# david-westreicher/minispark

Measured on AMD Instinct MI355X. Metric: TPC-H Q1 lineitem rows/sec, higher is better.
Workload: dtype f64

## Files before the change

minispark_amd/csrc/hs_agg_kernel.h:

```cpp
#pragma once

#include "hs_device.h"


typedef float hs_f32x4 __attribute__((ext_vector_type(4)));
typedef int hs_i32x4 __attribute__((ext_vector_type(4)));
typedef unsigned long long hs_u64x2 __attribute__((ext_vector_type(2)));

struct AggUnitArgs {
    hs_col key;
    hs_agg_spec spec;
    int32_t group_cap;
    int32_t hashed;
    int32_t batch;
    int32_t pad;
    const int64_t* unit_chunk0;
    const uint64_t* part_keys;
    const int64_t* part_rep;
    const uint64_t* part_acc;
    int64_t* out_rep;
    uint64_t* out_acc;
    int32_t* out_ngroups;
    uint32_t* flags;
    uint8_t* slab;
// ... 274 lines not shown
            const float4 v = *reinterpret_cast<const float4*>((const float*)c.data + row0);
            cell[0] = hs_d2u((double)v.x);
            cell[1] = hs_d2u((double)v.y);
            cell[2] = hs_d2u((double)v.z);
            cell[3] = hs_d2u((double)v.w);
            break;
        }
        case HS_I64:
        case HS_F64: {
            const ulonglong2 v0 = *reinterpret_cast<const ulonglong2*>((const uint64_t*)c.data + row0);
            const ulonglong2 v1 = *reinterpret_cast<const ulonglong2*>((const uint64_t*)c.data + row0 + 2);
            cell[0] = v0.x;
            cell[1] = v0.y;
            cell[2] = v1.x;
            cell[3] = v1.y;
            break;
        }
        case HS_U8: {
            const uint32_t v = *reinterpret_cast<const uint32_t*>((const uint8_t*)c.data + row0);
            cell[0] = v & 0xff;
            cell[1] = (v >> 8) & 0xff;
            cell[2] = (v >> 16) & 0xff;
            cell[3] = v >> 24;
            break;
        }
        case HS_I64_FOR16: {
            const uint2 v = *reinterpret_cast<const uint2*>((const uint16_t*)c.data + row0);
            const uint64_t b = (uint64_t)c.offs[0], s = (uint64_t)c.offs[1];
            cell[0] = b + (uint64_t)(v.x & 0xffff) * s;
            cell[1] = b + (uint64_t)(v.x >> 16) * s;
            cell[2] = b + (uint64_t)(v.y & 0xffff) * s;
            cell[3] = b + (uint64_t)(v.y >> 16) * s;
            break;
        }
        case HS_F32_LUT8: {
            const uint32_t v = *reinterpret_cast<const uint32_t*>((const uint8_t*)c.data + row0);
            const float* lut = (const float*)c.offs;
            const uint32_t last = (uint32_t)c.fixed_len - 1;
            cell[0] = hs_d2u((double)lut[min(v & 0xff, last)]);
            cell[1] = hs_d2u((double)lut[min((v >> 8) & 0xff, last)]);
            cell[2] = hs_d2u((double)lut[min((v >> 16) & 0xff, last)]);
            cell[3] = hs_d2u((double)lut[min(v >> 24, last)]);
            break;
        }
        case HS_STR:
            if (c.fixed_len == 1) hs_load_packed_quad<1>(c, row0, cell);
            else if (c.fixed_len == 2) hs_load_packed_quad<2>(c, row0, cell);
            else if (c.fixed_len == 4) hs_load_packed_quad<4>(c, row0, cell);
            break;
        default: break;
    }
}

struct AggCtx {
    int64_t row0;
    bool alive[HS_V];
    int slot[HS_V];
    uint64_t* dkeys;
    int64_t* dreps;
    uint64_t* tbl;
    uint8_t* dmap;
    uint32_t tid, nthr, mask;
    int32_t n_acc;
    uint32_t err;
    HsSpecBits sb;

    __device__ __forceinline__ int find_byte(const hs_col& key_col, uint64_t k, int64_t row, bool& live) {
        if (mask >= 255u) return find<false>(key_col, k, row, live);
        int s = 0;
        if (live) {
            const uint32_t b = (uint32_t)k & 0xffu;
            s = dmap[b];
            if (s == 0xff) {
                s = hs_dict_upsert_word(dkeys, dreps, mask, k, row);
                if (s < 0) {
                    err |= HS_FLAG_DICT_FULL;
                    live = false;
                    s = 0;
                } else {
                    dmap[b] = (uint8_t)s;
                }
            }
        }
        return s;
    }

    template <bool HASHED>
    __device__ __forceinline__ int find(const hs_col& key_col, uint64_t k, int64_t row, bool& live) {
        int s = 0;
        if (live) {
            if constexpr (HASHED) s = hs_dict_upsert_rows(dreps, mask, key_col, k, row);
            else s = hs_dict_upsert_word(dkeys, dreps, mask, k, row);
            if (s < 0) {
                err |= HS_FLAG_DICT_FULL;
                live = false;
                s = 0;
            }
        }
        return s;
    }

    __device__ __forceinline__ void fold(const hs_agg_spec& spec, uint32_t a, int s, bool live, uint64_t x) {
        if (live) {
            const uint32_t idx = ((uint32_t)s * (uint32_t)n_acc + a) * nthr + tid;
            (void)spec;
            tbl[idx] = hs_acc_fold(hs_spec_op(sb, a), hs_spec_int(sb, a), tbl[idx], x);
        }
    }

    template <int NA, int A, int OP, bool IS_INT>
    __device__ __forceinline__ void fold_c(int s, bool live, uint64_t x) {
        const uint32_t idx = ((uint32_t)(live ? s : 0) * (uint32_t)NA + (uint32_t)A) * nthr + tid;
        const uint64_t v = live ? x : hs_acc_identity(OP, IS_INT);
        tbl[idx] = hs_acc_fold(OP, IS_INT, tbl[idx], v);
    }
};

template <bool HASHED_, int D>
struct InterpProg {
    static constexpr bool HASHED = HASHED_;
    static constexpr bool TWO_STAGE = false;
    static constexpr bool STATIC_SPEC = false;
    static constexpr int NA = 0;
    static constexpr bool HAS_TABLES = false;
    struct Tables {};
    static __device__ constexpr uint32_t acc_op(int) { return 0; }
    static __device__ constexpr bool acc_int(int) { return false; }
    struct Cells {
        uint64_t cell[HS_FUSED_COLS][HS_V];
    };

    static __device__ __forceinline__ void load(const AggMainArgs& A, int64_t base, Cells& x) {
        const int ncols = A.cols.n < HS_FUSED_COLS ? A.cols.n : HS_FUSED_COLS;
#pragma unroll
        for (int c = 0; c < HS_FUSED_COLS; ++c) {
            if (c < ncols) {
                const hs_col& col = A.cols.c[c];
                if (col.kind != HS_STR || (c == A.key_col && hs_str_preloads(col))) hs_load_quad(col, base, x.cell[c]);
            }
        }
    }

    template <class Ctx>
    struct Sink {
        const AggMainArgs& A;
        const Cells& x;
        Ctx& ctx;
        __device__ __forceinline__ Sink(const AggMainArgs& a, const Cells& c, Ctx& k) : A(a), x(c), ctx(k) {}
        __device__ __forceinline__ void load(uint32_t s, uint64_t (&dst)[HS_V]) const {
            switch (s) {
#define HS_CASE(K)                                                          \
    case K:                                                                 \
        _Pragma("unroll") for (int j = 0; j < HS_V; ++j) dst[j] = x.cell[K][j]; \
        break;
                HS_CASE(0) HS_CASE(1) HS_CASE(2) HS_CASE(3) HS_CASE(4) HS_CASE(5) HS_CASE(6) HS_CASE(7)
#undef HS_CASE
                default: break;
            }
        }
        __device__ __forceinline__ uint64_t load(uint32_t s, int j) const {
            uint64_t tmp[HS_V];
            load(s, tmp);
            return tmp[j];
        }
        __device__ __forceinline__ bool live(int j) const { return ctx.alive[j]; }
        __device__ __forceinline__ int64_t row(int j) const { return ctx.row0 + j; }
        __device__ __forceinline__ void filter(int j, bool keep) { ctx.alive[j] = ctx.alive[j] && keep; }
        __device__ __forceinline__ void out(uint32_t, int, uint64_t) {}
        __device__ __forceinline__ void key() {
            const hs_col& kc = A.cols.c[A.key_col];
            uint64_t kcell[HS_V];
            const bool pre = (kc.kind != HS_STR) || hs_str_preloads(kc);
            if (pre) load((uint32_t)A.key_col, kcell);
            uint64_t ucell[HS_V] = {0, 0, 0, 0};
            if (A.unit_col >= 0) load((uint32_t)A.unit_col, ucell);
#pragma unroll
            for (int j = 0; j < HS_V; ++j) {
// ... 91 lines not shown
    extern __shared__ __align__(16) uint64_t hs_lds[];
    const uint32_t tid = threadIdx.x, nthr = blockDim.x;
    const int GC = A.group_cap;
    const int NA = A.spec.n_acc;
    uint64_t* dkeys = hs_lds;
    int64_t* dreps = (int64_t*)(hs_lds + GC);
    uint64_t* tbl = hs_lds + 2 * GC;

    const int64_t chunk = blockIdx.x;
    HS_SCAN_STAMP(0);
    if (A.stamps && threadIdx.x == 0)
        A.stamps[chunk * 16 + 7] = ((int64_t)__builtin_amdgcn_s_getreg((32 - 1) << 11 | 20) << 32) |
                                  (int64_t)(uint32_t)__builtin_amdgcn_s_getreg((32 - 1) << 11 | 4);
    const hs_chunk desc = A.chunks[chunk];
    const int64_t us = desc.unit_begin, c0 = desc.row_begin, c1 = desc.row_end;
    const int64_t stride = (int64_t)nthr * HS_V;
    int64_t base = c0 + (int64_t)tid * HS_V;
    typename Prog::Cells cur, nxt;
    if (base < c1) Prog::load(A, base, nxt);
    typename Prog::Tables tv;
    if constexpr (Prog::HAS_TABLES) Prog::load_tables(A, tid, tv);
    const HsSpecBits sb = hs_spec_bits(A.spec);

    __shared__ uint32_t s_overflowed;
    if (threadIdx.x == 0) s_overflowed = __hip_atomic_load(A.flags, __ATOMIC_RELAXED, __HIP_MEMORY_SCOPE_AGENT) & HS_FLAG_DICT_FULL;
    for (int i = tid; i < GC; i += nthr) {
        dkeys[i] = HS_EMPTY_KEY;
        dreps[i] = -1;
    }
    __shared__ uint8_t s_dmap[256];
    for (int i = tid; i < 256; i += nthr) s_dmap[i] = 0xff;
    for (int cellid = 0; cellid < GC * NA; ++cellid)
        tbl[(uint32_t)cellid * nthr + tid] = hs_acc_identity(hs_spec_op(sb, cellid % NA), hs_spec_int(sb, cellid % NA));
    if constexpr (Prog::HAS_TABLES) Prog::store_tables(tv, tid);
    __syncthreads();
    HS_SCAN_STAMP(1);
    if (s_overflowed) {
        for (int i = threadIdx.x; i < A.group_cap; i += blockDim.x) {
            hs_st_part(&A.part_keys[chunk * A.group_cap + i], HS_EMPTY_KEY);
            hs_st_part(&A.part_rep[chunk * A.group_cap + i], (int64_t)-1);
        }
    } else {
    AggCtx ctx;
    ctx.dkeys = dkeys;
    ctx.dreps = dreps;
    ctx.tbl = tbl;
    ctx.dmap = s_dmap;
    ctx.tid = tid;
    ctx.nthr = nthr;
    ctx.mask = (uint32_t)GC - 1;
    ctx.n_acc = NA;
    ctx.err = 0;
    ctx.sb = sb;
    HS_SCAN_STAMP(2);

    while (base < c1) {
        cur = nxt;
        const int64_t next_base = base + stride;
        if (next_base < c1) Prog::load(A, next_base, nxt);
        ctx.row0 = base;
#pragma unroll
        for (int j = 0; j < HS_V; ++j) {
            const int64_t r = base + j;
            ctx.alive[j] = (r >= us) && (r < c1);
            ctx.slot[j] = 0;
        }
        Prog::run(A, cur, ctx);
        base = next_base;
    }
    HS_SCAN_STAMP(3);
    __syncthreads();
    HS_SCAN_STAMP(14);

    const uint32_t wave = (uint32_t)__builtin_amdgcn_readfirstlane((int)(tid / HS_WAVE)), lane = tid % HS_WAVE, nwaves = nthr / HS_WAVE;
    if constexpr (Prog::STATIC_SPEC && (Prog::NA > 0)) {
        constexpr int SNA = Prog::NA;
        for (uint32_t sl = wave; sl < (uint32_t)GC; sl += nwaves) {
            if (__builtin_amdgcn_readfirstlane((int)(dreps[sl] >= 0)) == 0) continue;
            uint64_t v[SNA], t[SNA];
#pragma unroll
            for (int a = 0; a < SNA; ++a) v[a] = hs_acc_identity(Prog::acc_op(a), Prog::acc_int(a));
            for (uint32_t t0 = lane; t0 < nthr; t0 += HS_WAVE) {
#pragma unroll
                for (int a = 0; a < SNA; ++a) t[a] = tbl[(sl * (uint32_t)SNA + (uint32_t)a) * nthr + t0];
#pragma unroll
                for (int a = 0; a < SNA; ++a) v[a] = hs_acc_fold(Prog::acc_op(a), Prog::acc_int(a), v[a], t[a]);
            }
#pragma unroll
            for (int d = HS_WAVE / 2; d >= 1; d >>= 1) {
#pragma unroll
                for (int a = 0; a < SNA; ++a) t[a] = hs_shfl_down64(v[a], d);
#pragma unroll
                for (int a = 0; a < SNA; ++a) v[a] = hs_acc_fold(Prog::acc_op(a), Prog::acc_int(a), v[a], t[a]);
            }
            if (lane == 0) {
#pragma unroll
                for (int a = 0; a < SNA; ++a) hs_st_part(&A.part_acc[((int64_t)chunk * GC + sl) * SNA + a], v[a]);
            }
        }
    } else {
    constexpr int HS_RED = 6;
    const uint32_t ncells = (uint32_t)(GC * NA);
    for (uint32_t c0id = wave; c0id < ncells; c0id += nwaves * HS_RED) {
        uint64_t v[HS_RED], t[HS_RED];
        uint32_t ops[HS_RED];
        bool ints[HS_RED], on[HS_RED];
#pragma unroll
        for (int k = 0; k < HS_RED; ++k) {
            const uint32_t cellid = c0id + (uint32_t)k * nwaves;
            on[k] = cellid < ncells && __builtin_amdgcn_readfirstlane((int)(dreps[cellid < ncells ? cellid / NA : 0] >= 0)) != 0;
            const uint32_t a = on[k] ? cellid % NA : 0;
            ops[k] = hs_spec_op(sb, a);
            ints[k] = hs_spec_int(sb, a);
            v[k] = hs_acc_identity(ops[k], ints[k]);
        }
        for (uint32_t t0 = lane; t0 < nthr; t0 += HS_WAVE) {
#pragma unroll
            for (int k = 0; k < HS_RED; ++k) t[k] = on[k] ? tbl[(c0id + (uint32_t)k * nwaves) * nthr + t0] : 0ull;
#pragma unroll
            for (int k = 0; k < HS_RED; ++k)
                if (on[k]) v[k] = hs_acc_fold(ops[k], ints[k], v[k], t[k]);
// ... 446 lines not shown
```

minispark_amd/csrc/hs_jit.hip:

```cpp
#include <hip/hip_runtime.h>
#include <hip/hiprtc.h>
#include <stdarg.h>
#include <stdio.h>
#include <stdlib.h>
#include <string.h>

#include <chrono>
#include <mutex>
#include <string>
#include <sys/stat.h>
#include <unistd.h>

#include <unordered_map>
#include <vector>

#include "hs_agg_kernel.h"
#include "hs_embed.inc"

void hs_set_error(const char* fmt, ...);

namespace {

struct JitEntry {
    hipModule_t module = nullptr;
    hipFunction_t fn = nullptr;
    bool failed = false;
};

std::mutex g_mu;
std::unordered_map<std::string, JitEntry> g_cache;
int g_enabled = -1;
int g_compiled = 0, g_launches = 0, g_failures = 0;
std::string g_last_log;

bool jit_enabled() {
    if (g_enabled < 0) {
        const char* e = getenv("HIPSPARK_JIT");
        g_enabled = (e && e[0] == '0') ? 0 : 1;
    }
    return g_enabled != 0;
}

void appendf(std::string& s, const char* fmt, ...) {
    char buf[512];
    va_list ap;
    va_start(ap, fmt);
    vsnprintf(buf, sizeof(buf), fmt, ap);
    va_end(ap);
    s += buf;
}

bool slot_preloaded(const AggMainArgs& A, int c) {
    if (c >= A.cols.n || c >= HS_FUSED_COLS) return false;
    const hs_col& col = A.cols.c[c];
    if (col.kind != HS_STR) return true;
    return c == A.key_col && (col.fixed_len == 1 || col.fixed_len == 2 || col.fixed_len == 4);
}

int lut_entries(const hs_col& col) {
    int n = 16;
    while (n < col.fixed_len && n < 256) n *= 2;
    return n;
}

std::string cache_key(const AggMainArgs& A, bool hashed, bool shared, int nthr, bool scalar = false) {
    std::string k;
    int dev = 0;
    (void)hipGetDevice(&dev);
    appendf(k, "d%d|", dev);
    appendf(k, "v13|s%d|h%d|n%d|k%d|u%d|w%d|", shared ? 1 : scalar ? 2 : 0, hashed ? 1 : 0, A.cols.n, A.key_col, A.unit_col, shared ? 0 : nthr);
    for (int c = 0; c < A.cols.n; ++c) {
        const hs_col& col = A.cols.c[c];
        int fl = -1;
        if (col.kind == HS_STR && (col.fixed_len == 1 || col.fixed_len == 2 || col.fixed_len == 4) && c == A.key_col)
            fl = col.fixed_len;
        if (col.kind == HS_F32_LUT8) fl = lut_entries(col);
        appendf(k, "c%d:%d:%d|", c, col.kind, fl);
    }
    appendf(k, "a%d|", A.spec.n_acc);
    for (int a = 0; a < A.spec.n_acc; ++a) appendf(k, "%d%d", A.spec.op[a], A.spec.is_int[a]);
    k += "|";
    for (uint32_t i = 0; i < A.prog.n_ins; ++i) appendf(k, "%llx,", (unsigned long long)A.prog.ins[i]);
    return k;
}

std::string packed_cell_expr(const hs_col& col, int slot) {
    std::string e;

    if (col.kind == HS_U8) appendf(e, "((x.c%d_w[0] >> (8 * j)) & 0xffu)", slot);
    else if (col.fixed_len == 1) appendf(e, "((1ull << 56) | ((x.c%d_w[0] >> (8 * j)) & 0xffu))", slot);
    else if (col.fixed_len == 2) appendf(e, "((2ull << 56) | ((x.c%d_w[j >> 1] >> (16 * (j & 1))) & 0xffffu))", slot);
    else appendf(e, "((4ull << 56) | x.c%d_w[j])", slot);
    return e;
}

std::string ld_expr(const AggMainArgs& A, int slot) {
    std::string e;
    switch (A.cols.c[slot].kind & ~HS_PAIR) {
        case HS_I32: appendf(e, "(unsigned long long)(long long)x.c%d[j]", slot); break;
        case HS_F32: appendf(e, "hs_d2u((double)x.c%d[j])", slot); break;
        case HS_U8: e = "(unsigned long long)" + packed_cell_expr(A.cols.c[slot], slot); break;
        case HS_I64_FOR16:
            appendf(e, "(for%d_b + (unsigned long long)((unsigned)(x.c%d_q >> (16 * j)) & 0xffffu) * for%d_s)", slot, slot, slot);
            break;
        case HS_F32_LUT8:
            appendf(e, "hs_d2u(hs_lut_c%d[(x.c%d_w[0] >> (8 * j)) & %uu])", slot, slot, (unsigned)lut_entries(A.cols.c[slot]) - 1);
            break;
        case HS_JOIN8_CODE: e = "(unsigned long long)vb[j]"; break;
        case HS_JOIN8_UNIT: e = "(unsigned long long)vu[j]"; break;
        default: appendf(e, "x.c%d[j]", slot); break;
    }
    return e;
}


bool generate(const AggMainArgs& A, bool hashed, std::string& src, std::string& why, bool shared = false, int nthr = 256,
              bool scalar = false) {
    if (scalar && (shared || hashed || A.key_col >= 0 || A.unit_col >= 0)) {
        why = "the keyless kernel takes no key, unit column or shared table";
        return false;
    }
    const int NA = A.spec.n_acc;
    std::vector<std::string> agg_value((size_t)(NA > 0 ? NA : 0));
    const char* LD4 = "__builtin_nontemporal_load";
    std::string cells, loads, key_loads, join_prologue, body, hoisted, pair_keys, pair_take;
    std::string tables, table_regs, table_load, table_init;
    int j8_code = -1, j8_unit = -1, j8_src = -1;
    for (int c = 0; c < A.cols.n && c < HS_FUSED_COLS; ++c) {
        if (!slot_preloaded(A, c)) continue;
        const hs_col& col = A.cols.c[c];
        switch (col.kind) {
            case HS_I32:
                appendf(cells, "    int c%d[4];\n", c);
                appendf(loads, "    { const hs_i32x4 v = %s(reinterpret_cast<const hs_i32x4*>((const int*)A.cols.c[%d].data + base)); "
                               "x.c%d[0] = v.x; x.c%d[1] = v.y; x.c%d[2] = v.z; x.c%d[3] = v.w; }\n", LD4, c, c, c, c, c);
                break;
            case HS_F32:
                appendf(cells, "    float c%d[4];\n", c);
                appendf(loads, "    { const hs_f32x4 v = %s(reinterpret_cast<const hs_f32x4*>((const float*)A.cols.c[%d].data + base)); "
                               "x.c%d[0] = v.x; x.c%d[1] = v.y; x.c%d[2] = v.z; x.c%d[3] = v.w; }\n", LD4, c, c, c, c, c);
                break;
            case HS_I64:
            case HS_F64:
                appendf(cells, "    unsigned long long c%d[4];\n", c);
                appendf(loads, "    { const hs_u64x2 v0 = %s(reinterpret_cast<const hs_u64x2*>((const unsigned long long*)A.cols.c[%d].data + base)); "
                               "const hs_u64x2 v1 = %s(reinterpret_cast<const hs_u64x2*>((const unsigned long long*)A.cols.c[%d].data + base + 2)); "
                               "x.c%d[0] = v0.x; x.c%d[1] = v0.y; x.c%d[2] = v1.x; x.c%d[3] = v1.y; }\n", LD4, c, LD4, c, c, c, c, c);
                break;
            case HS_U8:
                appendf(cells, "    unsigned c%d_w[1];\n", c);
                appendf(loads, "    x.c%d_w[0] = *reinterpret_cast<const unsigned*>((const unsigned char*)A.cols.c[%d].data + base);\n", c, c);
                break;
            case HS_I64_FOR16:
            case HS_F32_LUT8:
                if (shared || c == A.key_col || c == A.unit_col || !col.offs || (col.kind == HS_F32_LUT8 && (col.fixed_len < 1 || col.fixed_len > 256))) {
                    why = "narrow columns are argument slots of the private-table and keyless tiers";
                    return false;
                }
                if (col.kind == HS_I64_FOR16) {
                    appendf(cells, "    unsigned long long c%d_q;\n", c);
                    appendf(loads, "    x.c%d_q = %s(reinterpret_cast<const unsigned long long*>((const unsigned short*)A.cols.c[%d].data + base));\n", c, LD4, c);
                    appendf(tables, "__shared__ unsigned long long hs_for_c%d[2];\n", c);
                    appendf(table_regs, "    unsigned long long for%d;\n", c);
                    appendf(table_load, "    t.for%d = (unsigned long long)A.cols.c[%d].offs[tid & 1u];\n", c, c);
                    appendf(table_init, "    if (tid < 2) hs_for_c%d[tid] = t.for%d;\n", c, c);
                    appendf(hoisted, "    const unsigned long long for%d_b = hs_for_c%d[0], for%d_s = hs_for_c%d[1];\n", c, c, c, c);
                } else {
                    const int entries = lut_entries(col);
                    appendf(cells, "    unsigned c%d_w[1];\n", c);
                    appendf(loads, "    x.c%d_w[0] = %s(reinterpret_cast<const unsigned*>((const unsigned char*)A.cols.c[%d].data + base));\n", c, LD4, c);
                    appendf(tables, "__shared__ double hs_lut_c%d[%d];\n", c, entries);
                    for (int k = 0; k * nthr < entries; ++k) {
                        appendf(table_regs, "    float lut%d_%d;\n", c, k);
                        appendf(table_load, "    t.lut%d_%d = ((const float*)A.cols.c[%d].offs)[min(tid + %du, (unsigned)A.cols.c[%d].fixed_len - 1u)];\n",
                                c, k, c, (unsigned)(k * nthr), c);
                        appendf(table_init, "    if (tid + %du < %du) hs_lut_c%d[tid + %du] = (double)t.lut%d_%d;\n", (unsigned)(k * nthr),
                                (unsigned)entries, c, (unsigned)(k * nthr), c, k);
                    }
                }
                break;
            case HS_STR:
                appendf(cells, "    unsigned c%d_w[%d];\n", c, col.fixed_len);
                if (col.fixed_len == 1)
                    appendf(loads, "    x.c%d_w[0] = *reinterpret_cast<const unsigned*>((const unsigned char*)A.cols.c[%d].data + base);\n", c, c);
                else if (col.fixed_len == 2)
                    appendf(loads, "    { const uint2 v = *reinterpret_cast<const uint2*>((const unsigned char*)A.cols.c[%d].data + base * 2); "
                                   "x.c%d_w[0] = v.x; x.c%d_w[1] = v.y; }\n", c, c, c);
                else
                    appendf(loads, "    { const uint4 v = *reinterpret_cast<const uint4*>((const unsigned char*)A.cols.c[%d].data + base * 4); "
                                   "x.c%d_w[0] = v.x; x.c%d_w[1] = v.y; x.c%d_w[2] = v.z; x.c%d_w[3] = v.w; }\n", c, c, c, c, c);
                break;
            case HS_JOIN8_CODE:
            case HS_JOIN8_UNIT:
                if (col.kind == HS_JOIN8_CODE) j8_code = c; else j8_unit = c;
                j8_src = c;
                break;
            case HS_PAIR | HS_I32:
            case HS_PAIR | HS_F32:
            case HS_PAIR | HS_I64: {
                if (!shared || c == A.key_col) {
                    why = "HS_PAIR columns are argument slots of the shared tier";
                    return false;
                }
                const int base = col.kind & ~HS_PAIR;
                const char* ty = base == HS_I32 ? "int" : base == HS_F32 ? "float" : "unsigned long long";
                appendf(cells, "    %s c%d[4];\n    long long ix%d[4];\n", ty, c, c);
                appendf(pair_keys, "    { const hs_u64x2 i0 = %s(reinterpret_cast<const hs_u64x2*>(A.cols.c[%d].offs + base)); "
                                   "const hs_u64x2 i1 = %s(reinterpret_cast<const hs_u64x2*>(A.cols.c[%d].offs + base + 2));\n"
                                   "      x.ix%d[0] = (long long)i0.x; x.ix%d[1] = (long long)i0.y; x.ix%d[2] = (long long)i1.x; "
                                   "x.ix%d[3] = (long long)i1.y; }\n", LD4, c, LD4, c, c, c, c, c);
                appendf(loads, "    { const %s* d = (const %s*)A.cols.c[%d].data; x.c%d[0] = d[x.ix%d[0]]; x.c%d[1] = d[x.ix%d[1]]; "
                               "x.c%d[2] = d[x.ix%d[2]]; x.c%d[3] = d[x.ix%d[3]]; }\n", ty, ty, c, c, c, c, c, c, c, c, c);
                appendf(pair_take, "    x.ix%d[0] = k.ix%d[0]; x.ix%d[1] = k.ix%d[1]; x.ix%d[2] = k.ix%d[2]; x.ix%d[3] = k.ix%d[3];\n",
                        c, c, c, c, c, c, c, c);
                break;
            }
            default:
                why = "unsupported column kind";
                return false;
        }
    }
    if (j8_src >= 0) {
        if (!shared || A.unit_col != j8_unit || j8_unit < 0 || !A.join.table) {
            why = "HS_JOIN8_* columns need the shared tier with the HS_JOIN8_UNIT column as unit column";
            return false;
        }
        cells += "    int jk[4];\n    unsigned jb[4];\n";
        appendf(key_loads, "    { const hs_i32x4 kv = %s(reinterpret_cast<const hs_i32x4*>((const int*)A.cols.c[%d].data + base));\n"
                           "      x.jk[0] = kv.x; x.jk[1] = kv.y; x.jk[2] = kv.z; x.jk[3] = kv.w; }\n", LD4, j8_src);
        loads += "    x.jb[0] = hs_join8_lookup(A.join, x.jk[0]);\n";
        loads += "    x.jb[1] = x.jk[1] != x.jk[0] ? hs_join8_lookup(A.join, x.jk[1]) : 0u;\n";
        loads += "    x.jb[2] = x.jk[2] != x.jk[1] ? hs_join8_lookup(A.join, x.jk[2]) : 0u;\n";
        loads += "    x.jb[3] = x.jk[3] != x.jk[2] ? hs_join8_lookup(A.join, x.jk[3]) : 0u;\n";
        join_prologue += "    unsigned vb[4], vu[4];\n    { const int np = A.join.n_parts;\n      const double inv = 1.0 / (double)np;\n";
        join_prologue += "      vb[0] = x.jb[0];\n      vu[0] = vb[0] == 0xffu ? 0xffu : hs_py_partition_inv(x.jk[0], np, inv);\n";
        for (int j = 1; j < 4; ++j) {
            appendf(join_prologue, "      { const bool same = x.jk[%d] == x.jk[%d];\n        vb[%d] = same ? vb[%d] : x.jb[%d];\n", j, j - 1, j, j - 1, j);
            appendf(join_prologue, "        vu[%d] = same ? vu[%d] : (vb[%d] == 0xffu ? 0xffu : hs_py_partition_inv(x.jk[%d], np, inv)); }\n", j, j - 1, j, j);
        }
        join_prologue += "    }\n";
    }
    key_loads += pair_keys;
    if (cells.empty()) cells = "    int unused;\n";

    std::vector<std::string> st;
    int tmp = 0;
    bool have_key = false;
    auto push_tmp = [&](const std::string& expr) {
        appendf(body, "        const unsigned long long t%d = %s;\n", tmp, expr.c_str());
        std::string name;
        appendf(name, "t%d", tmp++);
        st.push_back(name);
    };
    for (uint32_t pc = 0; pc < A.prog.n_ins; ++pc) {
        const uint64_t w = A.prog.ins[pc];
        const uint32_t op = (uint32_t)(w & 0xff), a = (uint32_t)((w >> 16) & 0xffff), b = (uint32_t)((w >> 32) & 0xffff),
                       c = (uint32_t)((w >> 48) & 0xffff);
        if (((w >> 8) & 0xff) != st.size()) {
            why = "stack depth annotation does not match";
            return false;
        }
        std::string e;
        const bool str_op = op == HS_OP_STRCMP_LIT || op == HS_OP_STRCMP_COL || op == HS_OP_LIKE || op == HS_OP_DICTBIT;
        if ((str_op && (int)a < A.cols.n && (A.cols.c[a].kind & HS_PAIR)) ||
            (op == HS_OP_STRCMP_COL && (int)b < A.cols.n && (A.cols.c[b].kind & HS_PAIR)) ||
            (op == HS_OP_KEY && (A.cols.c[A.key_col].kind & HS_PAIR))) {
            why = "an HS_PAIR column read as a string, a dictionary code or the key";
            return false;
        }
        if (op == HS_OP_LD) {
            if ((int)a >= A.cols.n || !slot_preloaded(A, (int)a) || A.cols.c[a].kind == HS_STR) {
                why = "LD of a column that is not preloaded";
                return false;
            }
            push_tmp(ld_expr(A, (int)a));
        } else if (op == HS_OP_LIT) {
            std::string name;
            appendf(name, "k%d", tmp++);
            appendf(hoisted, "    const unsigned long long %s = A.prog.lit[%u];\n", name.c_str(), a);
            st.push_back(name);
        } else if (op >= HS_OP_ADD_F && op <= HS_OP_OR) {
            if (st.size() < 2) { why = "stack underflow"; return false; }
            const std::string y = st.back(); st.pop_back();
            const std::string x = st.back(); st.pop_back();
            appendf(e, "hs_bin<%u>(%s, %s, live, ctx.err)", op, x.c_str(), y.c_str());
            push_tmp(e);
        } else if (op == HS_OP_I2F) {
            if (st.size() < (a ? 2u : 1u)) { why = "stack underflow"; return false; }
            const size_t idx = st.size() - 1 - (a ? 1 : 0);
            appendf(e, "hs_d2u((double)(long long)%s)", st[idx].c_str());
            std::string name;
            if (st[idx][0] == 'k') {
                appendf(name, "k%d", tmp++);
                appendf(hoisted, "    const unsigned long long %s = %s;\n", name.c_str(), e.c_str());
            } else {
                appendf(name, "t%d", tmp++);
                appendf(body, "        const unsigned long long %s = %s;\n", name.c_str(), e.c_str());
            }
            st[idx] = name;
        } else if (op == HS_OP_SEL) {
            if (st.size() < 3) { why = "stack underflow"; return false; }
            const std::string y = st.back(); st.pop_back();
            const std::string x = st.back(); st.pop_back();
            const std::string cnd = st.back(); st.pop_back();
            appendf(e, "(%s != 0 ? %s : %s)", cnd.c_str(), x.c_str(), y.c_str());
            if (cnd[0] == 'k' && x[0] == 'k' && y[0] == 'k') {
                std::string name;
                appendf(name, "k%d", tmp++);
                appendf(hoisted, "    const unsigned long long %s = %s;\n", name.c_str(), e.c_str());
                st.push_back(name);
            } else {
                push_tmp(e);
            }
        } else if (op == HS_OP_DATEPART) {
            if (st.empty()) { why = "stack underflow"; return false; }
            if (!(a <= HS_DP_DAYOFYEAR || (a >= HS_DT_YEAR && a <= HS_DT_SECOND))) { why = "DATEPART selector out of range"; return false; }
            const std::string x = st.back(); st.pop_back();
            appendf(e, "hs_datepart_c<%uu>(%s)", a, x.c_str());
            if (x[0] == 'k') {
                std::string name;
                appendf(name, "k%d", tmp++);
                appendf(hoisted, "    const unsigned long long %s = %s;\n", name.c_str(), e.c_str());
                st.push_back(name);
            } else {
                push_tmp(e);
            }
        } else if (op == HS_OP_STRCMP_LIT) {
            appendf(e, "(live ? hs_strcmp_lit(A.prog, A.cols.c[%u], r, %u, %u) : 0ull)", a, b, c);
            push_tmp(e);
        } else if (op == HS_OP_STRCMP_COL) {
            appendf(e, "(live ? hs_strcmp_col(A.cols.c[%u], A.cols.c[%u], r, %u) : 0ull)", a, b, c);
            push_tmp(e);
        } else if (op == HS_OP_LIKE) {
            appendf(e, "(live ? hs_like_lit(A.prog, A.cols.c[%u], r, %u) : 0ull)", a, b);
            push_tmp(e);
        } else if (op == HS_OP_DICTBIT) {
            if ((int)a < A.cols.n && A.cols.c[a].kind == HS_U8 && slot_preloaded(A, (int)a))
                appendf(e, "hs_dictbit_code(A.prog, %s, %u, %u)", packed_cell_expr(A.cols.c[a], (int)a).c_str(), b, c);
            else
                appendf(e, "(live ? hs_dictbit(A.prog, A.cols.c[%u], r, %u, %u) : 0ull)", a, b, c);
            push_tmp(e);
        } else if (op == HS_OP_FILTER) {
            if (st.empty()) { why = "stack underflow"; return false; }
            appendf(body, "        live = live && (%s != 0);\n", st.back().c_str());
            st.pop_back();
        } else if (op == HS_OP_KEY) {
            if (scalar) { why = "KEY in a keyless program"; return false; }
            const int K = A.key_col;
            const hs_col& kc = A.cols.c[K];
            std::string kexpr;
            if (kc.kind == HS_JOIN8_CODE) kexpr = "(unsigned long long)vb[j]";
            else if (kc.kind != HS_STR) appendf(kexpr, "hs_key_from_cell(%d, %s)", kc.kind, ld_expr(A, K).c_str());
            else if (slot_preloaded(A, K)) kexpr = packed_cell_expr(kc, K);
            else appendf(kexpr, "(live ? hs_key_at(A.cols.c[%d], r) : 0ull)", K);
            if (A.unit_col >= 0) {
                const int U = A.unit_col;
                if (U >= A.cols.n || !slot_preloaded(A, U) || (A.cols.c[U].kind != HS_U8 && A.cols.c[U].kind != HS_JOIN8_UNIT) || hashed) {
                    why = "unit column must be a preloaded HS_U8 slot next to a packing key";
                    return false;
                }
                std::string uref;
                if (A.cols.c[U].kind == HS_JOIN8_UNIT) uref = "vu[j]";
                else uref = packed_cell_expr(A.cols.c[U], U);
                appendf(body, "        live = live && %s != 0xffu;\n", uref.c_str());
                hoisted += "    unsigned long long prev_kw = 0;\n    int prev_slot = 0;\n    bool prev_live = false;\n";
                appendf(body, "        const unsigned long long kw = hs_unit_key(%s, %s);\n", kexpr.c_str(), uref.c_str());
                appendf(body, "        int slot;\n        if (live && prev_live && kw == prev_kw) slot = prev_slot;\n"
                              "        else slot = ctx.template find<HASHED>(A.cols.c[%d], kw, r, live);\n", K);
                body += "        prev_kw = kw; prev_slot = slot; prev_live = live;\n";
            } else if (!hashed && kc.kind == HS_STR && kc.fixed_len == 1)
                appendf(body, "        const int slot = ctx.find_byte(A.cols.c[%d], %s, r, live);\n", K, kexpr.c_str());
            else
                appendf(body, "        const int slot = ctx.template find<HASHED>(A.cols.c[%d], %s, r, live);\n", K, kexpr.c_str());
            have_key = true;
        } else if (op == HS_OP_AGG) {
            if (st.empty() || (!have_key && !scalar) || (int)a >= NA) { why = "AGG before KEY or bad accumulator"; return false; }
            if (!agg_value[a].empty()) { why = "accumulator fed twice"; return false; }
            agg_value[a] = st.back();
            st.pop_back();
        } else {
            why = "opcode not covered by the translator";
            return false;
        }
    }
    if (!st.empty()) { why = "unbalanced program"; return false; }
    std::string post;
    if (shared && NA > 0) {
        if (!have_key) { why = "aggregates without a key"; return false; }
        for (int a = 0; a < NA; ++a) {
            if (agg_value[a].empty()) { why = "accumulator never fed"; return false; }
        }
        hoisted += "    int run_slot = 0;\n    bool run_live = false;\n";
        for (int a = 0; a < NA; ++a) appendf(hoisted, "    unsigned long long run_a%d = 0;\n", a);
        std::string flush;
        for (int a = 0; a < NA; ++a)
            appendf(flush, "ctx.template fold_c<%d, %d, %d, %s>(run_slot, true, run_a%d); ", NA, a, (int)A.spec.op[a],
                    A.spec.is_int[a] ? "true" : "false", a);
        appendf(body, "        if (live) {\n            if (run_live && slot == run_slot) {\n");
        for (int a = 0; a < NA; ++a)
            appendf(body, "                run_a%d = hs_acc_fold(%d, %s, run_a%d, %s);\n", a, (int)A.spec.op[a],
                    A.spec.is_int[a] ? "true" : "false", a, agg_value[a].c_str());
        body += "            } else {\n                if (run_live) { " + flush + "}\n                run_slot = slot;\n                run_live = true;\n";
        for (int a = 0; a < NA; ++a) appendf(body, "                run_a%d = %s;\n", a, agg_value[a].c_str());
        appendf(body, "            }\n        }\n");
        post += "    if (run_live) { " + flush + "}\n";
    }
    if (scalar) {
        for (int a = 0; a < NA; ++a) {
            if (agg_value[a].empty()) { why = "accumulator never fed"; return false; }
            appendf(body, "        ctx.acc[%d] = hs_acc_fold(%d, %s, ctx.acc[%d], live ? %s : hs_acc_identity(%d, %s));\n", a,
                    (int)A.spec.op[a], A.spec.is_int[a] ? "true" : "false", a, agg_value[a].c_str(), (int)A.spec.op[a],
                    A.spec.is_int[a] ? "true" : "false");
        }
        body += "        ctx.rows += live ? 1 : 0;\n";
    }
    if (!shared && !scalar && NA > 0) {
        if (!have_key) { why = "aggregates without a key"; return false; }
        appendf(body, "        if (live) {\n");
        appendf(body, "            uint64_t* cell = ctx.tbl + (unsigned)slot * %uu + ctx.tid;\n", (unsigned)(NA * nthr));
        for (int a = 0; a < NA; ++a)
            if (!agg_value[a].empty()) appendf(body, "            uint64_t a%d = cell[%u];\n", a, (unsigned)(a * nthr));
        for (int a = 0; a < NA; ++a)
            if (!agg_value[a].empty())
                appendf(body, "            a%d = hs_acc_fold(%d, %s, a%d, %s);\n", a, (int)A.spec.op[a],
                        A.spec.is_int[a] ? "true" : "false", a, agg_value[a].c_str());
        for (int a = 0; a < NA; ++a)
            if (!agg_value[a].empty()) appendf(body, "            cell[%u] = a%d;\n", (unsigned)(a * nthr), a);
        appendf(body, "        }\n");
    }

    src.clear();
    src += "#include \"hs_agg_kernel.h\"\n";
    src += tables;
    src += "struct JitProg {\n";
    appendf(src, "  static constexpr bool HAS_TABLES = %s;\n", tables.empty() ? "false" : "true");
    src += "  struct Tables {\n" + table_regs + "  };\n";
    if (!tables.empty()) {
        src += "  static __device__ __forceinline__ void load_tables(const AggMainArgs& A, unsigned tid, Tables& t) {\n" + table_load + "  }\n";
        src += "  static __device__ __forceinline__ void store_tables(const Tables& t, unsigned tid) {\n" + table_init + "  }\n";
    }
    appendf(src, "  static constexpr bool HASHED = %s;\n", hashed ? "true" : "false");
    appendf(src, "  static constexpr bool TWO_STAGE = %s;\n", key_loads.empty() ? "false" : "true");
    {
        std::string ops = "0u", ints = "false";
        for (int a = NA - 1; a >= 0; --a) {
            char buf[64];
            snprintf(buf, sizeof buf, "a == %d ? %uu : ", a, (unsigned)A.spec.op[a]);
            ops = std::string(buf) + ops;
            snprintf(buf, sizeof buf, "a == %d ? %s : ", a, A.spec.is_int[a] ? "true" : "false");
            ints = std::string(buf) + ints;
        }
        appendf(src, "  static constexpr bool STATIC_SPEC = true;\n  static constexpr int NA = %d;\n", NA > 0 ? NA : 0);
        src += "  static __device__ constexpr uint32_t acc_op(int a) { return " + ops + "; }\n";
        src += "  static __device__ constexpr bool acc_int(int a) { return " + ints + "; }\n";
    }
    src += "  struct Cells {\n" + cells + "  };\n";
    src += "  static __device__ __forceinline__ void load(const AggMainArgs& A, int64_t base, Cells& x) {\n" + loads + "  }\n";
    if (!key_loads.empty()) {
        src += "  static __device__ __forceinline__ void load_keys(const AggMainArgs& A, int64_t base, Cells& x) {\n" + key_loads + "  }\n";
        src += "  static __device__ __forceinline__ void take_keys(Cells& x, const Cells& k) {\n";
        if (j8_src >= 0) src += "    x.jk[0] = k.jk[0]; x.jk[1] = k.jk[1]; x.jk[2] = k.jk[2]; x.jk[3] = k.jk[3];\n";
        src += pair_take + "  }\n";
    }
    src += "  template <class Ctx>\n  static __device__ __forceinline__ void run(const AggMainArgs& A, const Cells& x, Ctx& ctx) {\n";
    src += join_prologue;
    src += hoisted;
    src += "#pragma unroll\n";
    src += "    for (int j = 0; j < HS_V; ++j) {\n";
    src += "        bool live = ctx.alive[j];\n";
    src += "        const int64_t r = ctx.row0 + j;\n";
    src += "        (void)r;\n";
    src += body;
    src += "    }\n";
    src += post;
    src += "  }\n};\n";
    if (scalar) {
        appendf(src, "extern \"C\" __global__ void __launch_bounds__(%d) k_agg_scalar_jit(const AggMainArgs A_kernarg) {\n", nthr);
        src += "    HS_KERNARG(AggMainArgs, A);\n";
        src += "    hs_agg_scalar_body<JitProg>(A);\n}\n";
    } else if (shared) {
        src += "extern \"C\" __global__ void __launch_bounds__(1024) k_agg_shared_jit(const AggMainArgs A_kernarg) {\n";
        src += "    HS_KERNARG(AggMainArgs, A);\n";
        src += "    hs_agg_shared_body<JitProg>(A);\n}\n";
    } else {
        appendf(src, "extern \"C\" __global__ void __launch_bounds__(%d) k_agg_jit(const AggMainArgs A_kernarg) {\n", nthr);
        src += "    HS_KERNARG(AggMainArgs, A);\n";
        appendf(src, "    if (blockDim.x != %du) { if (threadIdx.x == 0) atomicOr(A.flags, HS_FLAG_BAD_PROGRAM); return; }\n", nthr);
        src += "    hs_agg_main_body<JitProg>(A);\n}\n";
    }
    return true;
}

std::string eval_cache_key(const EvalArgs& A) {
    std::string k;
    int dev = 0;
    (void)hipGetDevice(&dev);
    appendf(k, "d%d|eval2|n%d|", dev, A.cols.n);
    for (int c = 0; c < A.cols.n; ++c) appendf(k, "c%d:%d|", c, A.cols.c[c].kind);
    for (int o = 0; o < HS_MAX_OUTS; ++o) appendf(k, "%d", A.out_kinds[o]);
    k += "|";
    for (uint32_t i = 0; i < A.prog.n_ins; ++i) appendf(k, "%llx,", (unsigned long long)A.prog.ins[i]);
    return k;
}

bool generate_eval(const EvalArgs& A, std::string& src, std::string& why) {
    const char* LD4 = "__builtin_nontemporal_load";
    bool used[HS_MAX_COLS] = {};
    bool out_used[HS_MAX_OUTS] = {};
    for (uint32_t pc = 0; pc < A.prog.n_ins; ++pc) {
        const uint64_t w = A.prog.ins[pc];
        const uint32_t op = (uint32_t)(w & 0xff), a = (uint32_t)((w >> 16) & 0xffff);
        if (op == HS_OP_LD) {
            if ((int)a >= A.cols.n || A.cols.c[a].kind == HS_STR) { why = "LD of a string or missing column"; return false; }
            used[a] = true;
        }
    }
    std::string cells, loads, body, stores;
    for (int c = 0; c < A.cols.n; ++c) {
        if (!used[c]) continue;
        switch (A.cols.c[c].kind) {
            case HS_I32:
                appendf(cells, "        int c%d[4];\n", c);
                appendf(loads, "        { const hs_i32x4 v = %s(reinterpret_cast<const hs_i32x4*>((const int*)A.cols.c[%d].data + base)); "
                               "c%d[0] = v.x; c%d[1] = v.y; c%d[2] = v.z; c%d[3] = v.w; }\n", LD4, c, c, c, c, c);
                break;
            case HS_F32:
                appendf(cells, "        float c%d[4];\n", c);
                appendf(loads, "        { const hs_f32x4 v = %s(reinterpret_cast<const hs_f32x4*>((const float*)A.cols.c[%d].data + base)); "
                               "c%d[0] = v.x; c%d[1] = v.y; c%d[2] = v.z; c%d[3] = v.w; }\n", LD4, c, c, c, c, c);
                break;
            case HS_I64:
            case HS_F64:
                appendf(cells, "        unsigned long long c%d[4];\n", c);
                appendf(loads, "        { const hs_u64x2 v0 = %s(reinterpret_cast<const hs_u64x2*>((const unsigned long long*)A.cols.c[%d].data + base)); "
                               "const hs_u64x2 v1 = %s(reinterpret_cast<const hs_u64x2*>((const unsigned long long*)A.cols.c[%d].data + base + 2)); "
                               "c%d[0] = v0.x; c%d[1] = v0.y; c%d[2] = v1.x; c%d[3] = v1.y; }\n", LD4, c, LD4, c, c, c, c, c);
                break;
            case HS_U8:
                appendf(cells, "        unsigned c%d[4];\n", c);
                appendf(loads, "        { const unsigned v = *reinterpret_cast<const unsigned*>((const unsigned char*)A.cols.c[%d].data + base); "
// ... 479 lines not shown
```

Measured before the change: 411.8 billion.

## Specialize JIT aggregation: interior steps, FOR16 threshold compares, batched byte-key lookup

Adds an interior-step context whose rows are all known to be alive, so the generated kernel can skip the per-row bounds masks. Comparisons between FOR16-encoded columns and literals become compares on the raw 16-bit codes against thresholds precomputed per block, which avoids decoding those values. Single-byte string keys are looked up in a batched pass through the dmap, falling back to a slow path only when some lane misses, and LUT8 values are decoded together in one batch. Accumulator cells are addressed through an LDS pointer with __umul24. The cost is more complex code generation, a new cache version, and an extra group_cap guard that rejects batched kernels when the cap is too large.

```diff
diff --git a/minispark_amd/csrc/hs_agg_kernel.h b/minispark_amd/csrc/hs_agg_kernel.h
--- a/minispark_amd/csrc/hs_agg_kernel.h
+++ b/minispark_amd/csrc/hs_agg_kernel.h
@@ -350,6 +350,15 @@
     }
 }
 
+__device__ __forceinline__ uint32_t hs_for16_threshold(int64_t base, int64_t scale, int64_t lit, bool strict) {
+    if (strict ? lit <= base : lit < base) return 0u;
+    const uint64_t diff = (uint64_t)lit - (uint64_t)base;
+    const uint64_t s = scale < 1 ? 1ull : (uint64_t)scale;
+    const uint64_t q = diff / s;
+    if (q >= 65536ull) return 65536u;
+    return (uint32_t)q + (strict ? (diff % s != 0 ? 1u : 0u) : 1u);
+}
+
 struct AggCtx {
     int64_t row0;
     bool alive[HS_V];
@@ -362,9 +371,9 @@
     int32_t n_acc;
     uint32_t err;
     HsSpecBits sb;
-
-    __device__ __forceinline__ int find_byte(const hs_col& key_col, uint64_t k, int64_t row, bool& live) {
-        if (mask >= 255u) return find<false>(key_col, k, row, live);
+    static constexpr bool ALL_ALIVE = false;
+
+    __device__ __forceinline__ int find_byte_small(uint64_t k, int64_t row, bool& live) {
         int s = 0;
         if (live) {
             const uint32_t b = (uint32_t)k & 0xffu;
@@ -383,6 +392,11 @@
         return s;
     }
 
+    __device__ __forceinline__ int find_byte(const hs_col& key_col, uint64_t k, int64_t row, bool& live) {
+        if (mask >= 255u) return find<false>(key_col, k, row, live);
+        return find_byte_small(k, row, live);
+    }
+
     template <bool HASHED>
     __device__ __forceinline__ int find(const hs_col& key_col, uint64_t k, int64_t row, bool& live) {
         int s = 0;
@@ -414,6 +428,10 @@
     }
 };
 
+struct AggCtxInterior : AggCtx {
+    static constexpr bool ALL_ALIVE = true;
+};
+
 template <bool HASHED_, int D>
 struct InterpProg {
     static constexpr bool HASHED = HASHED_;
@@ -421,6 +439,7 @@
     static constexpr bool STATIC_SPEC = false;
     static constexpr int NA = 0;
     static constexpr bool HAS_TABLES = false;
+    static constexpr bool INTERIOR_STEPS = false;
     struct Tables {};
     static __device__ constexpr uint32_t acc_op(int) { return 0; }
     static __device__ constexpr bool acc_int(int) { return false; }
@@ -618,21 +637,39 @@
     ctx.n_acc = NA;
     ctx.err = 0;
     ctx.sb = sb;
+#pragma unroll
+    for (int j = 0; j < HS_V; ++j) {
+        ctx.alive[j] = false;
+        ctx.slot[j] = 0;
+    }
     HS_SCAN_STAMP(2);
 
+    int64_t step_begin = c0;
     while (base < c1) {
         cur = nxt;
         const int64_t next_base = base + stride;
         if (next_base < c1) Prog::load(A, next_base, nxt);
         ctx.row0 = base;
-#pragma unroll
-        for (int j = 0; j < HS_V; ++j) {
-            const int64_t r = base + j;
-            ctx.alive[j] = (r >= us) && (r < c1);
-            ctx.slot[j] = 0;
-        }
-        Prog::run(A, cur, ctx);
+        bool interior = false;
+        if constexpr (Prog::INTERIOR_STEPS) interior = us <= step_begin && step_begin + stride <= c1;
+        if (interior) {
+            if constexpr (Prog::INTERIOR_STEPS) {
+                AggCtxInterior ictx;
+                static_cast<AggCtx&>(ictx) = ctx;
+                Prog::run(A, cur, ictx);
+                ctx.err = ictx.err;
+            }
+        } else {
+#pragma unroll
+            for (int j = 0; j < HS_V; ++j) {
+                const int64_t r = base + j;
+                ctx.alive[j] = (r >= us) && (r < c1);
+                ctx.slot[j] = 0;
+            }
+            Prog::run(A, cur, ctx);
+        }
         base = next_base;
+        step_begin += stride;
     }
     HS_SCAN_STAMP(3);
     __syncthreads();
diff --git a/minispark_amd/csrc/hs_jit.hip b/minispark_amd/csrc/hs_jit.hip
--- a/minispark_amd/csrc/hs_jit.hip
+++ b/minispark_amd/csrc/hs_jit.hip
@@ -68,7 +68,7 @@
     int dev = 0;
     (void)hipGetDevice(&dev);
     appendf(k, "d%d|", dev);
-    appendf(k, "v13|s%d|h%d|n%d|k%d|u%d|w%d|", shared ? 1 : scalar ? 2 : 0, hashed ? 1 : 0, A.cols.n, A.key_col, A.unit_col, shared ? 0 : nthr);
+    appendf(k, "v14|s%d|h%d|n%d|k%d|u%d|w%d|", shared ? 1 : scalar ? 2 : 0, hashed ? 1 : 0, A.cols.n, A.key_col, A.unit_col, shared ? 0 : nthr);
     for (int c = 0; c < A.cols.n; ++c) {
         const hs_col& col = A.cols.c[c];
         int fl = -1;
@@ -126,6 +126,10 @@
     std::string cells, loads, key_loads, join_prologue, body, hoisted, pair_keys, pair_take;
     std::string tables, table_regs, table_load, table_init;
     int j8_code = -1, j8_unit = -1, j8_src = -1;
+    struct ForCmp { int slot; uint32_t lit; bool strict; };
+    std::vector<int> for_slots;
+    std::vector<ForCmp> for_cmp;
+    bool for_decoded[HS_FUSED_COLS] = {};
     for (int c = 0; c < A.cols.n && c < HS_FUSED_COLS; ++c) {
         if (!slot_preloaded(A, c)) continue;
         const hs_col& col = A.cols.c[c];
@@ -160,11 +164,7 @@
                 if (col.kind == HS_I64_FOR16) {
                     appendf(cells, "    unsigned long long c%d_q;\n", c);
                     appendf(loads, "    x.c%d_q = %s(reinterpret_cast<const unsigned long long*>((const unsigned short*)A.cols.c[%d].data + base));\n", c, LD4, c);
-                    appendf(tables, "__shared__ unsigned long long hs_for_c%d[2];\n", c);
-                    appendf(table_regs, "    unsigned long long for%d;\n", c);
-                    appendf(table_load, "    t.for%d = (unsigned long long)A.cols.c[%d].offs[tid & 1u];\n", c, c);
-                    appendf(table_init, "    if (tid < 2) hs_for_c%d[tid] = t.for%d;\n", c, c);
-                    appendf(hoisted, "    const unsigned long long for%d_b = hs_for_c%d[0], for%d_s = hs_for_c%d[1];\n", c, c, c, c);
+                    for_slots.push_back(c);
                 } else {
                     const int entries = lut_entries(col);
                     appendf(cells, "    unsigned c%d_w[1];\n", c);
@@ -252,6 +252,31 @@
         appendf(name, "t%d", tmp++);
         st.push_back(name);
     };
+    std::unordered_map<std::string, uint32_t> lit_of;
+    auto val = [&](const std::string& name) -> std::string {
+        if (name[0] != 'F') return name;
+        const int slot = atoi(name.c_str() + 1);
+        for_decoded[slot] = true;
+        std::string t;
+        appendf(t, "t%d", tmp++);
+        appendf(body, "        const unsigned long long %s = %s;\n", t.c_str(), ld_expr(A, slot).c_str());
+        return t;
+    };
+    bool batched = false;
+    std::string pre, lut_batch, batched_key;
+    bool lut_batched[HS_FUSED_COLS] = {};
+    if (!shared && !scalar && !hashed && A.unit_col < 0 && NA > 0 && A.key_col >= 0 && A.key_col < A.cols.n &&
+        A.cols.c[A.key_col].kind == HS_STR && A.cols.c[A.key_col].fixed_len == 1 && slot_preloaded(A, A.key_col) &&
+        (144 * 1024) / (8 * NA * nthr) < 255) {
+        int keys = 0;
+        bool ok = true;
+        for (uint32_t pc = 0; pc < A.prog.n_ins; ++pc) {
+            const uint32_t op = (uint32_t)(A.prog.ins[pc] & 0xff);
+            if (op == HS_OP_KEY) ok = ok && ++keys == 1 && ((A.prog.ins[pc] >> 8) & 0xff) == 0;
+            if (op == HS_OP_FILTER && keys) ok = false;
+        }
+        batched = ok && keys == 1;
+    }
     for (uint32_t pc = 0; pc < A.prog.n_ins; ++pc) {
         const uint64_t w = A.prog.ins[pc];
         const uint32_t op = (uint32_t)(w & 0xff), a = (uint32_t)((w >> 16) & 0xffff), b = (uint32_t)((w >> 32) & 0xffff),
@@ -273,21 +298,52 @@
                 why = "LD of a column that is not preloaded";
                 return false;
             }
-            push_tmp(ld_expr(A, (int)a));
+            if (A.cols.c[a].kind == HS_I64_FOR16) {
+                std::string name;
+                appendf(name, "F%u", a);
+                st.push_back(name);
+            } else if (batched && have_key && A.cols.c[a].kind == HS_F32_LUT8) {
+                if (!lut_batched[a]) {
+                    lut_batched[a] = true;
+                    appendf(lut_batch, "    double lut%u_q[HS_V];\n#pragma unroll\n    for (int j = 0; j < HS_V; ++j) lut%u_q[j] = "
+                                       "hs_lut_c%u[(x.c%u_w[0] >> (8 * j)) & %uu];\n", a, a, a, a, (unsigned)lut_entries(A.cols.c[a]) - 1);
+                }
+                appendf(e, "hs_d2u(lut%u_q[j])", a);
+                push_tmp(e);
+            } else {
+                push_tmp(ld_expr(A, (int)a));
+            }
         } else if (op == HS_OP_LIT) {
             std::string name;
             appendf(name, "k%d", tmp++);
             appendf(hoisted, "    const unsigned long long %s = A.prog.lit[%u];\n", name.c_str(), a);
+            lit_of[name] = a;
             st.push_back(name);
         } else if (op >= HS_OP_ADD_F && op <= HS_OP_OR) {
             if (st.size() < 2) { why = "stack underflow"; return false; }
-            const std::string y = st.back(); st.pop_back();
-            const std::string x = st.back(); st.pop_back();
-            appendf(e, "hs_bin<%u>(%s, %s, live, ctx.err)", op, x.c_str(), y.c_str());
-            push_tmp(e);
+            std::string y = st.back(); st.pop_back();
+            std::string x = st.back(); st.pop_back();
+            const bool fx = x[0] == 'F', fy = y[0] == 'F';
+            if (op >= HS_OP_LT_I && op <= HS_OP_GE_I && fx != fy && lit_of.count(fx ? y : x)) {
+                const uint32_t vop = fx ? op : op == HS_OP_LT_I ? HS_OP_GT_I : op == HS_OP_LE_I ? HS_OP_GE_I : op == HS_OP_GT_I ? HS_OP_LT_I : HS_OP_LE_I;
+                const int slot = atoi((fx ? x : y).c_str() + 1);
+                const bool strict = vop == HS_OP_LT_I || vop == HS_OP_GE_I;
+                const bool below = vop == HS_OP_LT_I || vop == HS_OP_LE_I;
+                int n_of_slot = 0;
+                for (const ForCmp& f : for_cmp) n_of_slot += f.slot == slot ? 1 : 0;
+                appendf(e, "(unsigned long long)(((unsigned)(x.c%d_q >> (16 * j)) & 0xffffu) %s for%d_t%d)", slot, below ? "<" : ">=", slot, n_of_slot);
+                for_cmp.push_back({slot, lit_of[fx ? y : x], strict});
+                push_tmp(e);
+            } else {
+                x = val(x);
+                y = val(y);
+                appendf(e, "hs_bin<%u>(%s, %s, live, ctx.err)", op, x.c_str(), y.c_str());
+                push_tmp(e);
+            }
         } else if (op == HS_OP_I2F) {
             if (st.size() < (a ? 2u : 1u)) { why = "stack underflow"; return false; }
             const size_t idx = st.size() - 1 - (a ? 1 : 0);
+            st[idx] = val(st[idx]);
             appendf(e, "hs_d2u((double)(long long)%s)", st[idx].c_str());
             std::string name;
             if (st[idx][0] == 'k') {
@@ -300,9 +356,9 @@
             st[idx] = name;
         } else if (op == HS_OP_SEL) {
             if (st.size() < 3) { why = "stack underflow"; return false; }
-            const std::string y = st.back(); st.pop_back();
-            const std::string x = st.back(); st.pop_back();
-            const std::string cnd = st.back(); st.pop_back();
+            const std::string y = val(st.back()); st.pop_back();
+            const std::string x = val(st.back()); st.pop_back();
+            const std::string cnd = val(st.back()); st.pop_back();
             appendf(e, "(%s != 0 ? %s : %s)", cnd.c_str(), x.c_str(), y.c_str());
             if (cnd[0] == 'k' && x[0] == 'k' && y[0] == 'k') {
                 std::string name;
@@ -315,7 +371,7 @@
         } else if (op == HS_OP_DATEPART) {
             if (st.empty()) { why = "stack underflow"; return false; }
             if (!(a <= HS_DP_DAYOFYEAR || (a >= HS_DT_YEAR && a <= HS_DT_SECOND))) { why = "DATEPART selector out of range"; return false; }
-            const std::string x = st.back(); st.pop_back();
+            const std::string x = val(st.back()); st.pop_back();
             appendf(e, "hs_datepart_c<%uu>(%s)", a, x.c_str());
             if (x[0] == 'k') {
                 std::string name;
@@ -342,7 +398,7 @@
             push_tmp(e);
         } else if (op == HS_OP_FILTER) {
             if (st.empty()) { why = "stack underflow"; return false; }
-            appendf(body, "        live = live && (%s != 0);\n", st.back().c_str());
+            appendf(body, "        live = live && (%s != 0);\n", val(st.back()).c_str());
             st.pop_back();
         } else if (op == HS_OP_KEY) {
             if (scalar) { why = "KEY in a keyless program"; return false; }
@@ -368,6 +424,9 @@
                 appendf(body, "        int slot;\n        if (live && prev_live && kw == prev_kw) slot = prev_slot;\n"
                               "        else slot = ctx.template find<HASHED>(A.cols.c[%d], kw, r, live);\n", K);
                 body += "        prev_kw = kw; prev_slot = slot; prev_live = live;\n";
+            } else if (batched) {
+                pre.swap(body);
+                batched_key = kexpr;
             } else if (!hashed && kc.kind == HS_STR && kc.fixed_len == 1)
                 appendf(body, "        const int slot = ctx.find_byte(A.cols.c[%d], %s, r, live);\n", K, kexpr.c_str());
             else
@@ -376,7 +435,7 @@
         } else if (op == HS_OP_AGG) {
             if (st.empty() || (!have_key && !scalar) || (int)a >= NA) { why = "AGG before KEY or bad accumulator"; return false; }
             if (!agg_value[a].empty()) { why = "accumulator fed twice"; return false; }
-            agg_value[a] = st.back();
+            agg_value[a] = val(st.back());
             st.pop_back();
         } else {
             why = "opcode not covered by the translator";
@@ -416,8 +475,10 @@
     }
     if (!shared && !scalar && NA > 0) {
         if (!have_key) { why = "aggregates without a key"; return false; }
+        hoisted += "    __attribute__((address_space(3))) uint64_t* const tbl_lds = (__attribute__((address_space(3))) uint64_t*)ctx.tbl;\n";
         appendf(body, "        if (live) {\n");
-        appendf(body, "            uint64_t* cell = ctx.tbl + (unsigned)slot * %uu + ctx.tid;\n", (unsigned)(NA * nthr));
+        appendf(body, "            __attribute__((address_space(3))) uint64_t* cell = tbl_lds + (__umul24((unsigned)slot, %uu) + ctx.tid);\n",
+                (unsigned)(NA * nthr));
         for (int a = 0; a < NA; ++a)
             if (!agg_value[a].empty()) appendf(body, "            uint64_t a%d = cell[%u];\n", a, (unsigned)(a * nthr));
         for (int a = 0; a < NA; ++a)
@@ -428,6 +489,29 @@
             if (!agg_value[a].empty()) appendf(body, "            cell[%u] = a%d;\n", (unsigned)(a * nthr), a);
         appendf(body, "        }\n");
     }
+    for (int c : for_slots) {
+        int n_cmp = 0;
+        for (const ForCmp& f : for_cmp) n_cmp += f.slot == c ? 1 : 0;
+        appendf(tables, "__shared__ unsigned long long hs_for_c%d[%d];\n", c, 2 + n_cmp);
+        appendf(table_regs, "    unsigned long long for%d;\n", c);
+        appendf(table_load, "    t.for%d = (unsigned long long)A.cols.c[%d].offs[tid & 1u];\n", c, c);
+        appendf(table_init, "    if (tid < 2) hs_for_c%d[tid] = t.for%d;\n", c, c);
+        if (for_decoded[c]) appendf(hoisted, "    const unsigned long long for%d_b = hs_for_c%d[0], for%d_s = hs_for_c%d[1];\n", c, c, c, c);
+        if (n_cmp) {
+            appendf(table_regs, "    long long for%d_scale;\n", c);
+            appendf(table_load, "    t.for%d_scale = A.cols.c[%d].offs[1];\n", c, c);
+        }
+        int k = 0;
+        for (const ForCmp& f : for_cmp) {
+            if (f.slot != c) continue;
+            appendf(table_regs, "    long long for%d_lit%d;\n", c, k);
+            appendf(table_load, "    t.for%d_lit%d = (long long)A.prog.lit[%u];\n", c, k, f.lit);
+            appendf(table_init, "    if (tid == 0) hs_for_c%d[%d] = hs_for16_threshold((long long)t.for%d, t.for%d_scale, t.for%d_lit%d, %s);\n",
+                    c, 2 + k, c, c, c, k, f.strict ? "true" : "false");
+            appendf(hoisted, "    const unsigned for%d_t%d = (unsigned)__builtin_amdgcn_readfirstlane((int)hs_for_c%d[%d]);\n", c, k, c, 2 + k);
+            ++k;
+        }
+    }
 
     src.clear();
     src += "#include \"hs_agg_kernel.h\"\n";
@@ -439,6 +523,7 @@
         src += "  static __device__ __forceinline__ void load_tables(const AggMainArgs& A, unsigned tid, Tables& t) {\n" + table_load + "  }\n";
         src += "  static __device__ __forceinline__ void store_tables(const Tables& t, unsigned tid) {\n" + table_init + "  }\n";
     }
+    appendf(src, "  static constexpr bool INTERIOR_STEPS = %s;\n", (shared || scalar) ? "false" : "true");
     appendf(src, "  static constexpr bool HASHED = %s;\n", hashed ? "true" : "false");
     appendf(src, "  static constexpr bool TWO_STAGE = %s;\n", key_loads.empty() ? "false" : "true");
     {
@@ -465,13 +550,34 @@
     src += "  template <class Ctx>\n  static __device__ __forceinline__ void run(const AggMainArgs& A, const Cells& x, Ctx& ctx) {\n";
     src += join_prologue;
     src += hoisted;
-    src += "#pragma unroll\n";
-    src += "    for (int j = 0; j < HS_V; ++j) {\n";
-    src += "        bool live = ctx.alive[j];\n";
-    src += "        const int64_t r = ctx.row0 + j;\n";
-    src += "        (void)r;\n";
-    src += body;
-    src += "    }\n";
+    const char* alive = (shared || scalar) ? "ctx.alive[j]" : "(Ctx::ALL_ALIVE || ctx.alive[j])";
+    if (batched) {
+        src += "    bool live_q[HS_V];\n    unsigned sraw[HS_V];\n    int slot_q[HS_V];\n";
+        src += "#pragma unroll\n    for (int j = 0; j < HS_V; ++j) {\n";
+        appendf(src, "        bool live = %s;\n", alive);
+        src += "        const int64_t r = ctx.row0 + j;\n        (void)r;\n";
+        src += pre;
+        src += "        live_q[j] = live;\n    }\n";
+        appendf(src, "#pragma unroll\n    for (int j = 0; j < HS_V; ++j) sraw[j] = ctx.dmap[(x.c%d_w[0] >> (8 * j)) & 0xffu];\n", A.key_col);
+        src += "    bool miss = false;\n#pragma unroll\n    for (int j = 0; j < HS_V; ++j) miss = miss || (live_q[j] && sraw[j] == 0xffu);\n";
+        src += "    if (__builtin_expect(__any(miss), 0)) {\n#pragma unroll\n        for (int j = 0; j < HS_V; ++j)\n";
+        appendf(src, "            slot_q[j] = ctx.find_byte_small(%s, ctx.row0 + j, live_q[j]);\n", batched_key.c_str());
+        src += "    } else {\n#pragma unroll\n        for (int j = 0; j < HS_V; ++j) slot_q[j] = (int)sraw[j];\n    }\n";
+        src += lut_batch;
+        src += "#pragma unroll\n    for (int j = 0; j < HS_V; ++j) {\n";
+        src += "        const bool live = live_q[j];\n        const int slot = slot_q[j];\n";
+        src += "        const int64_t r = ctx.row0 + j;\n        (void)r;\n";
+        src += body;
+        src += "    }\n";
+    } else {
+        src += "#pragma unroll\n";
+        src += "    for (int j = 0; j < HS_V; ++j) {\n";
+        appendf(src, "        bool live = %s;\n", alive);
+        src += "        const int64_t r = ctx.row0 + j;\n";
+        src += "        (void)r;\n";
+        src += body;
+        src += "    }\n";
+    }
     src += post;
     src += "  }\n};\n";
     if (scalar) {
@@ -485,7 +591,8 @@
     } else {
         appendf(src, "extern \"C\" __global__ void __launch_bounds__(%d) k_agg_jit(const AggMainArgs A_kernarg) {\n", nthr);
         src += "    HS_KERNARG(AggMainArgs, A);\n";
-        appendf(src, "    if (blockDim.x != %du) { if (threadIdx.x == 0) atomicOr(A.flags, HS_FLAG_BAD_PROGRAM); return; }\n", nthr);
+        appendf(src, "    if (blockDim.x != %du%s) { if (threadIdx.x == 0) atomicOr(A.flags, HS_FLAG_BAD_PROGRAM); return; }\n", nthr,
+                batched ? " || A.group_cap > 255" : "");
         src += "    hs_agg_main_body<JitProg>(A);\n}\n";
     }
     return true;
```

Result: faster. 437.2 billion, median of 6 (+6.2%).
